# mandt-lab/PSLD

Hardware: NVIDIA B200
Metric: PSLD CIFAR-10 samples/sec (SSCS sampler) (higher is better)
Workload: dtype bf16x3

## Files before the change

### psld_b200/csrc/attn_tc.cu

```cuda

#include <cuda.h>

#include <new>

#include "common.cuh"
#include "tc_common.cuh"
#include "conv_tc_common.cuh"

namespace psld {

constexpr int AT_TILE = 128 * 64 * 2;
constexpr int AT_RING = 3;

template <bool kX3>
struct AtCfg {
  static constexpr int kMul = kX3 ? 2 : 1;
  static constexpr int kQP = 4 * AT_TILE * kMul;
  static constexpr int kSlot = AT_TILE * kMul;
  static constexpr int kParts = kX3 ? 2 : 1;
  static constexpr int kThreads = 64 + 128 * kParts;
  static constexpr int kXchg = kX3 ? 2048 : 0;
  static constexpr int kSmem = kQP + AT_RING * kSlot + 256 + kXchg;
  static constexpr int kMinBlocks = kX3 ? 1 : 2;
};

#ifdef PSLD_TC_TRACE
__device__ long long g_at_trace[1024 * 8];
#define AT_TRACE(slot) do { if ((threadIdx.x & 31) == 0) { const int b_ = blockIdx.y * gridDim.x + blockIdx.x; if (b_ < 1024) g_at_trace[b_ * 8 + (slot)] = clock64(); } } while (0)
#else
#define AT_TRACE(slot) do { } while (0)
#endif

struct AttnTcParams {
  __nv_bfloat16* out;
  int HW, C, N;
  int q_rows;
  int k_rows;
  int w_rows;
  float scale_log2;
  ConvTcParams ep;
};

struct AttnTcState {
  CUtensorMap tq, tkv, tw;
  bool proj, x3;
  AttnTcParams p;
  dim3 grid;
};

template <bool kProj, bool kX3>
__global__ void __launch_bounds__(AtCfg<kX3>::kThreads, AtCfg<kX3>::kMinBlocks)
attn_tc_kernel(const __grid_constant__ CUtensorMap tmQ, const __grid_constant__ CUtensorMap tmKV,
               const __grid_constant__ CUtensorMap tmW, const AttnTcParams p) {
  using Cfg = AtCfg<kX3>;
  constexpr uint32_t QP_LO = 4u * AT_TILE;
  constexpr uint32_t S_LO = AT_TILE;
  extern __shared__ uint8_t smem_raw[];
  pdl_trigger_early();
  if (threadIdx.x == 0) AT_TRACE(0);
  const uint32_t base = smem_u32(smem_raw);
  if (base & 1023u) __trap();
  const uint32_t qp = base;
  const uint32_t ring = base + Cfg::kQP;
  const uint32_t bar_base = ring + AT_RING * Cfg::kSlot;
  auto full_bar = [&](int s) { return bar_base + 8u * s; };
  auto empty_bar = [&](int s) { return bar_base + 8u * (AT_RING + s); };
  const uint32_t q_full = bar_base + 8u * (2 * AT_RING);
  const uint32_t s_full = q_full + 8u;
  const uint32_t p_ready = q_full + 16u;
  const uint32_t o_full = q_full + 24u;
  const uint32_t o_ready = q_full + 32u;
  const uint32_t y_full = q_full + 40u;
  const uint32_t tmem_slot = q_full + 48u;
  const uint32_t stg_base = ring;
  const uint32_t addv_base = ring + 8u * 4096u;
  constexpr int kParts = Cfg::kParts;
  float* xchg = reinterpret_cast<float*>(smem_raw + (bar_base + 256u - base));
  volatile uint32_t* tmem_slot_ptr =
      reinterpret_cast<volatile uint32_t*>(smem_raw + (tmem_slot - base));

  const int warp = threadIdx.x >> 5, lane = threadIdx.x & 31;
  const int n = blockIdx.y, q0 = blockIdx.x * 128;
  const int nck = p.C / 64;
  const int nkh = (p.HW + 127) / 128;
  const int nwt = (p.C + 127) / 128;
  const int lo_c = 3 * p.C;

  if (warp == 0 && lane == 0) {
    asm volatile("prefetch.tensormap [%0];" ::"l"(&tmQ) : "memory");
    asm volatile("prefetch.tensormap [%0];" ::"l"(&tmKV) : "memory");
    if (kProj) asm volatile("prefetch.tensormap [%0];" ::"l"(&tmW) : "memory");
    for (int s = 0; s < AT_RING; ++s) {
      mbar_init(full_bar(s), 1);
      mbar_init(empty_bar(s), 1);
    }
    mbar_init(q_full, 1);
    mbar_init(s_full, 1);
    mbar_init(p_ready, 128 * kParts);
    mbar_init(o_full, 1);
    mbar_init(o_ready, 128 * kParts);
    mbar_init(y_full, 1);
    asm volatile("fence.mbarrier_init.release.cluster;" ::: "memory");
  }
  if (warp == 1) {
    asm volatile("tcgen05.alloc.cta_group::1.sync.aligned.shared::cta.b32 [%0], %1;"
                 ::"r"(tmem_slot), "n"(256) : "memory");
    asm volatile("tcgen05.relinquish_alloc_permit.cta_group::1.sync.aligned;" ::: "memory");
  }
  tc_fence_before();
  __syncthreads();
  tc_fence_after();
  pdl_wait();
  const uint32_t tmem_acc = *tmem_slot_ptr;

  if (warp == 0) {
    if (lane == 0) {
      const uint32_t mul = kX3 ? 2u : 1u;
      mbar_arrive_expect_tx(q_full, (uint32_t)(nck * p.q_rows) * 128u * mul);
      for (int c = 0; c < nck; ++c) {
        tma_load_3d(qp + (uint32_t)c * AT_TILE, &tmQ, q_full, c * 64, q0, n);
        if (kX3) tma_load_3d(qp + QP_LO + (uint32_t)c * AT_TILE, &tmQ, q_full, lo_c + c * 64, q0, n);
      }
      int slot = 0;
      uint32_t phase = 0;
      auto next = [&]() { if (++slot == AT_RING) { slot = 0; phase ^= 1; } };
      for (int c = 0; c < nck; ++c)
        for (int h = 0; h < nkh; ++h) {
          mbar_wait(empty_bar(slot), phase ^ 1);
          mbar_arrive_expect_tx(full_bar(slot), (uint32_t)p.k_rows * 128u * mul);
          const uint32_t st = ring + (uint32_t)slot * Cfg::kSlot;
          tma_load_3d(st, &tmKV, full_bar(slot), p.C + c * 64, h * 128, n);
          if (kX3) tma_load_3d(st + S_LO, &tmKV, full_bar(slot), lo_c + p.C + c * 64, h * 128, n);
          next();
        }
      for (int g = 0; g < nck; ++g)
        for (int h = 0; h < nkh; ++h) {
          mbar_wait(empty_bar(slot), phase ^ 1);
          mbar_arrive_expect_tx(full_bar(slot), (uint32_t)p.k_rows * 128u * mul);
          const uint32_t st = ring + (uint32_t)slot * Cfg::kSlot;
          tma_load_3d(st, &tmKV, full_bar(slot), 2 * p.C + g * 64, h * 128, n);
          if (kX3) tma_load_3d(st + S_LO, &tmKV, full_bar(slot), lo_c + 2 * p.C + g * 64, h * 128, n);
          next();
        }
      if (kProj) {
        for (int c = 0; c < nck; ++c)
          for (int t = 0; t < nwt; ++t) {
            mbar_wait(empty_bar(slot), phase ^ 1);
            mbar_arrive_expect_tx(full_bar(slot), (uint32_t)p.w_rows * 128u * mul);
            const uint32_t st = ring + (uint32_t)slot * Cfg::kSlot;
            tma_load_2d(st, &tmW, full_bar(slot), c * 64, t * 128);
            if (kX3) tma_load_2d(st + S_LO, &tmW, full_bar(slot), c * 64, p.C + t * 128);
            next();
          }
      }
    }
  } else if (warp == 1) {
    if (lane == 0) {
      int slot = 0;
      uint32_t phase = 0;
      auto next = [&]() { if (++slot == AT_RING) { slot = 0; phase ^= 1; } };
      auto kgroup = [&](uint32_t d, uint32_t a_hi, uint32_t b_hi, uint32_t a_lo, uint32_t b_lo, uint32_t idesc,
                        bool first) {
        const uint64_t ad = make_sw128_desc(a_hi), bd = make_sw128_desc(b_hi);
#pragma unroll
        for (int k = 0; k < 4; ++k)
          tc_mma_bf16(d, ad + (uint64_t)(2 * k), bd + (uint64_t)(2 * k), idesc, (!first || k > 0) ? 1u : 0u);
        if (kX3) {
          const uint64_t al = make_sw128_desc(a_lo), bl = make_sw128_desc(b_lo);
#pragma unroll
          for (int k = 0; k < 4; ++k) tc_mma_bf16(d, ad + (uint64_t)(2 * k), bl + (uint64_t)(2 * k), idesc, 1u);
#pragma unroll
          for (int k = 0; k < 4; ++k) tc_mma_bf16(d, al + (uint64_t)(2 * k), bd + (uint64_t)(2 * k), idesc, 1u);
        }
      };
      const uint32_t idesc_s = (1u << 4) | (1u << 7) | (1u << 10) | ((uint32_t)(p.k_rows >> 3) << 17) |
                               ((uint32_t)(128 >> 4) << 24);
      mbar_wait(q_full, 0);
      tc_fence_after();
      AT_TRACE(1);
      for (int c = 0; c < nck; ++c)
        for (int h = 0; h < nkh; ++h) {
          mbar_wait(full_bar(slot), phase);
          tc_fence_after();
          const uint32_t st = ring + (uint32_t)slot * Cfg::kSlot;
          kgroup(tmem_acc + (uint32_t)h * 128u, qp + (uint32_t)c * AT_TILE, st,
                 qp + QP_LO + (uint32_t)c * AT_TILE, st + S_LO, idesc_s, c == 0);
          tc_commit(empty_bar(slot));
          next();
        }
      tc_commit(s_full);
      const uint32_t idesc_o = (1u << 4) | (1u << 7) | (1u << 10) | (1u << 16) |
                               ((uint32_t)(64 >> 3) << 17) | ((uint32_t)(128 >> 4) << 24);
      mbar_wait(p_ready, 0);
      tc_fence_after();
      for (int g = 0; g < nck; ++g)
        for (int h = 0; h < nkh; ++h) {
          mbar_wait(full_bar(slot), phase);
          tc_fence_after();
          const uint32_t st = ring + (uint32_t)slot * Cfg::kSlot;
          const uint32_t d = tmem_acc + (uint32_t)g * 64u;
          for (int ks = 0; ks < p.k_rows / 16; ++ks) {
            const int kg = h * 8 + ks;
            const uint32_t pa = qp + (uint32_t)(kg >> 2) * AT_TILE;
            const uint64_t adesc = make_sw128_desc(pa) + (uint64_t)(2 * (kg & 3));
            const uint64_t bdesc = make_sw128_desc(st + (uint32_t)ks * 2048u);
            tc_mma_bf16(d, adesc, bdesc, idesc_o, (h > 0 || ks > 0) ? 1u : 0u);
            if (kX3) {
              const uint64_t adesc_lo = make_sw128_desc(pa + QP_LO) + (uint64_t)(2 * (kg & 3));
              const uint64_t bdesc_lo = make_sw128_desc(st + S_LO + (uint32_t)ks * 2048u);
              tc_mma_bf16(d, adesc, bdesc_lo, idesc_o, 1u);
              tc_mma_bf16(d, adesc_lo, bdesc, idesc_o, 1u);
            }
          }
          tc_commit(empty_bar(slot));
          next();
        }
      tc_commit(o_full);
      if (kProj) {
        mbar_wait(o_ready, 0);
        tc_fence_after();
        for (int c = 0; c < nck; ++c)
          for (int t = 0; t < nwt; ++t) {
            mbar_wait(full_bar(slot), phase);
            tc_fence_after();
            const int rows = (p.C - t * 128) < 128 ? (p.C - t * 128) : 128;
            const uint32_t idesc_y = (1u << 4) | (1u << 7) | (1u << 10) | ((uint32_t)(rows >> 3) << 17) |
                                     ((uint32_t)(128 >> 4) << 24);
            const uint32_t st = ring + (uint32_t)slot * Cfg::kSlot;
            kgroup(tmem_acc + (uint32_t)t * 128u, qp + (uint32_t)c * AT_TILE, st,
                   qp + QP_LO + (uint32_t)c * AT_TILE, st + S_LO, idesc_y, c == 0);
            tc_commit(empty_bar(slot));
            next();
          }
        tc_commit(y_full);
      }
    }
  } else {
    const int quarter = warp & 3;
    const int row = quarter * 32 + lane;
    const uint32_t lane_addr = (uint32_t)(quarter * 32) << 16;
    const int part = kParts == 2 ? (warp >= 6 ? 1 : 0) : 0;
    const int k_lo = part * (p.HW / kParts), k_hi = k_lo + p.HW / kParts;
    const int c_lo = part * (p.C / kParts), c_hi = c_lo + p.C / kParts;
    auto pair_sync = [&]() {
      if (kParts == 2) asm volatile("bar.sync %0, 64;" ::"r"(2 + quarter) : "memory");
    };
    mbar_wait(s_full, 0);
    tc_fence_after();
    if (warp == 2) AT_TRACE(2);
    float mx = -INFINITY;
    for (int ch = k_lo; ch < k_hi; ch += 32) {
      uint32_t r[32];
      tmem_ld32(tmem_acc + lane_addr + (uint32_t)ch, r);
      tmem_ld_wait();
#pragma unroll
      for (int j = 0; j < 32; ++j) mx = fmaxf(mx, __uint_as_float(r[j]));
    }
    if (kParts == 2) {
      xchg[part * 128 + row] = mx;
      pair_sync();
      mx = fmaxf(mx, xchg[(part ^ 1) * 128 + row]);
    }
    const float mxs = mx * p.scale_log2;
    float sum = 0.f;
    for (int ch = k_lo; ch < k_hi; ch += 32) {
      uint32_t r[32];
      tmem_ld32(tmem_acc + lane_addr + (uint32_t)ch, r);
      tmem_ld_wait();
      const uint32_t tile = qp + (uint32_t)(ch >> 6) * AT_TILE + (uint32_t)row * 128u;
      const int cbase = (ch & 63) >> 3;
#pragma unroll
      for (int q = 0; q < 4; ++q) {
        uint32_t w[4], wl[4];
#pragma unroll
        for (int t = 0; t < 4; ++t) {
          const float e0 = exp2f(fmaf(__uint_as_float(r[q * 8 + 2 * t]), p.scale_log2, -mxs));
          const float e1 = exp2f(fmaf(__uint_as_float(r[q * 8 + 2 * t + 1]), p.scale_log2, -mxs));
          if (kX3) {
            split_bf2(e0, e1, w[t], wl[t]);
            sum += e0 + e1;
          } else {
            __nv_bfloat162 h = __floats2bfloat162_rn(e0, e1);
            const float2 f = __bfloat1622float2(h);
            sum += f.x + f.y;
            w[t] = *reinterpret_cast<uint32_t*>(&h);
          }
        }
        const uint32_t dst = tile + (uint32_t)(((cbase + q) ^ (row & 7)) << 4);
        sts128(dst, w[0], w[1], w[2], w[3]);
        if (kX3) sts128(dst + QP_LO, wl[0], wl[1], wl[2], wl[3]);
      }
    }
    asm volatile("fence.proxy.async.shared::cta;" ::: "memory");
    tc_fence_before();
    mbar_arrive(p_ready);
    if (warp == 2) AT_TRACE(3);
    if (kParts == 2) {
      xchg[256 + part * 128 + row] = sum;
      pair_sync();
      sum += xchg[256 + (part ^ 1) * 128 + row];
    }
    const float inv = 1.0f / sum;
    mbar_wait(o_full, 0);
    tc_fence_after();
    if (warp == 2) AT_TRACE(4);
    const int q = q0 + row;
    const bool valid = q < p.HW;
    if (kProj) {
      for (int ch = c_lo; ch < c_hi; ch += 32) {
        uint32_t r[32];
        tmem_ld32(tmem_acc + lane_addr + (uint32_t)ch, r);
        tmem_ld_wait();
        const uint32_t tile = qp + (uint32_t)(ch >> 6) * AT_TILE + (uint32_t)row * 128u;
        const int cbase = (ch & 63) >> 3;
#pragma unroll
        for (int j = 0; j < 4; ++j) {
          uint32_t w[4], wl[4];
#pragma unroll
          for (int t = 0; t < 4; ++t) {
            const float o0 = __uint_as_float(r[j * 8 + 2 * t]) * inv;
            const float o1 = __uint_as_float(r[j * 8 + 2 * t + 1]) * inv;
            if (kX3) split_bf2(o0, o1, w[t], wl[t]);
            else w[t] = f2_to_bf2(o0, o1);
          }
          const uint32_t dst = tile + (uint32_t)(((cbase + j) ^ (row & 7)) << 4);
          sts128(dst, w[0], w[1], w[2], w[3]);
          if (kX3) sts128(dst + QP_LO, wl[0], wl[1], wl[2], wl[3]);
        }
      }
      asm volatile("fence.proxy.async.shared::cta;" ::: "memory");
      tc_fence_before();
      mbar_arrive(o_ready);
      if (warp == 2) AT_TRACE(5);
      mbar_wait(y_full, 0);
      tc_fence_after();
      if (warp == 2) AT_TRACE(6);
      const int m_tile = n * (p.HW >> 7) + (int)blockIdx.x;
      const int ew = warp - 2;
#pragma unroll 1
      for (int half = (kParts == 2 ? part : 0); half < (kParts == 2 ? part + 1 : 2); ++half)
        tc_epilogue_tile<true, kX3 ? 32 : 64, !kX3, kX3>(p.ep, tmem_acc, 0, m_tile, 0, p.ep.block_n, quarter, half, lane,
                                                         stg_base + (uint32_t)ew * 4096u,
                                                         addv_base + (uint32_t)ew * 256u, []() {}, []() {});
    } else {
      __nv_bfloat16* orow = p.out + ((int64_t)n * p.HW + q) * (p.C * (kX3 ? 2 : 1));
      for (int ch = c_lo; ch < c_hi; ch += 32) {
        uint32_t r[32];
        tmem_ld32(tmem_acc + lane_addr + (uint32_t)ch, r);
        tmem_ld_wait();
        if (valid) {
#pragma unroll
          for (int j = 0; j < 32; j += 8) {
            uint32_t w[4], wl[4];
#pragma unroll
            for (int t = 0; t < 4; ++t) {
              const float o0 = __uint_as_float(r[j + 2 * t]) * inv;
              const float o1 = __uint_as_float(r[j + 2 * t + 1]) * inv;
              if (kX3) split_bf2(o0, o1, w[t], wl[t]);
              else w[t] = f2_to_bf2(o0, o1);
            }
            *reinterpret_cast<uint4*>(orow + ch + j) = make_uint4(w[0], w[1], w[2], w[3]);
            if (kX3) *reinterpret_cast<uint4*>(orow + p.C + ch + j) = make_uint4(wl[0], wl[1], wl[2], wl[3]);
          }
        }
        __syncwarp();
      }
    }
  }

  tc_fence_before();
  __syncthreads();
  if (threadIdx.x == 0) AT_TRACE(7);
  if (warp == 1) {
    tc_fence_after();
    asm volatile("tcgen05.dealloc.cta_group::1.sync.aligned.b32 %0, %1;"
                 ::"r"(tmem_acc), "n"(256) : "memory");
  }
}

#ifdef PSLD_TC_TRACE
extern "C" __attribute__((visibility("default"))) int psld_debug_attn_trace(long long* out) {
  return cudaMemcpyFromSymbol(out, g_at_trace, sizeof(g_at_trace)) == cudaSuccess ? 0 : 1;
}
#endif

static int encode_qkv_map(CUtensorMap* tm, const void* ptr, int N, int HW, int C3, int rows) {
  const cuuint64_t dims[3] = {(cuuint64_t)C3, (cuuint64_t)HW, (cuuint64_t)N};
  const cuuint64_t strides[2] = {(cuuint64_t)C3 * 2, (cuuint64_t)HW * C3 * 2};
  const cuuint32_t box[3] = {64, (cuuint32_t)rows, 1};
  const cuuint32_t estr[3] = {1, 1, 1};
  return encode_bf16_map(tm, ptr, 3, dims, strides, box, estr, "qkv");
}

int prepare_attn_tc(psld_op& op) {
  const int N = op.i[PSLD_ATTN_N], HW = op.i[PSLD_ATTN_HW], C = op.i[PSLD_ATTN_C];
  auto unsupported = [&](const char* why) {
    set_error("attn_tc: not eligible (%s): N=%d HW=%d C=%d", why, N, HW, C);
    return PSLD_EUNSUPPORTED;
  };
  const int adt = op.i[PSLD_ATTN_DTYPE];
  if (adt != PSLD_BF16 && adt != PSLD_BF16S) return unsupported("dtype must be bf16 or split bf16");
  const bool x3 = adt == PSLD_BF16S;
  const int cm = x3 ? 2 : 1;
  if (C % 64 || C < 64 || C > 256) return unsupported("C must be 64..256, multiple of 64");
  if (HW != 64 && HW != 128 && HW != 256) return unsupported("HW must be 64, 128 or 256");
  if (!op.in[0] || !op.out[0]) { set_error("attn_tc: null pointer"); return PSLD_EINVAL; }
  AttnTcState* st = new (std::nothrow) AttnTcState();
  if (!st) { set_error("attn_tc: out of host memory"); return PSLD_ECUDA; }
  const int q_rows = HW < 128 ? HW : 128;
  st->x3 = x3;
  int rc = encode_qkv_map(&st->tq, op.in[0], N, HW, cm * 3 * C, q_rows);
  if (rc == PSLD_OK) rc = encode_qkv_map(&st->tkv, op.in[0], N, HW, cm * 3 * C, q_rows);
  if (rc != PSLD_OK) { delete st; return rc; }
  st->p.out = (__nv_bfloat16*)op.out[0];
  st->p.HW = HW; st->p.C = C; st->p.N = N; st->p.q_rows = q_rows;
  st->p.k_rows = q_rows; st->p.w_rows = C < 128 ? C : 128;
  st->p.scale_log2 = op.f[0] * 1.4426950408889634f;
  st->grid = dim3((unsigned)((HW + 127) / 128), (unsigned)N);
  st->proj = op.i[PSLD_ATTN_PROJ] != 0;
  if (st->proj) {
    if (HW % 128 || !op.in[1] || !op.in[3]) { delete st; return unsupported("fused projection needs HW %% 128 == 0, weight and residual"); }
    rc = encode_w_map(&st->tw, op.in[1], cm * C, C, C < 128 ? C : 128);
    if (rc != PSLD_OK) { delete st; return rc; }
    ConvTcParams& e = st->p.ep;
    e = ConvTcParams{};
    e.bias = (const float*)op.in[2];
    e.temb = nullptr;
    e.res = (const __nv_bfloat16*)op.in[3];
    e.y = (__nv_bfloat16*)op.out[0];
    e.y_nchw = nullptr;
    e.mg_stats = (double*)op.out[1];
    e.cout_valid = C;
    e.scale = op.f[1];
    e.HW = HW; e.Cout = C; e.H = 0; e.W = 0;
    e.block_n = C; e.n_tiles_n = 1;
    e.M = (int64_t)N * HW;
  } else {
    st->tw = st->tq;
  }
  static bool attr_set = false;
  if (!attr_set) {
    cudaError_t e = cudaFuncSetAttribute(attn_tc_kernel<false, false>,
                                         cudaFuncAttributeMaxDynamicSharedMemorySize, AtCfg<false>::kSmem);
    if (e == cudaSuccess)
      e = cudaFuncSetAttribute(attn_tc_kernel<true, false>, cudaFuncAttributeMaxDynamicSharedMemorySize,
                               AtCfg<false>::kSmem);
    if (e == cudaSuccess)
      e = cudaFuncSetAttribute(attn_tc_kernel<false, true>, cudaFuncAttributeMaxDynamicSharedMemorySize,
                               AtCfg<true>::kSmem);
    if (e == cudaSuccess)
      e = cudaFuncSetAttribute(attn_tc_kernel<true, true>, cudaFuncAttributeMaxDynamicSharedMemorySize,
                               AtCfg<true>::kSmem);
    if (e == cudaSuccess)
      e = cudaFuncSetAttribute(attn_tc_kernel<false, false>, cudaFuncAttributePreferredSharedMemoryCarveout, 100);
    if (e == cudaSuccess)
      e = cudaFuncSetAttribute(attn_tc_kernel<true, false>, cudaFuncAttributePreferredSharedMemoryCarveout, 100);
    if (e != cudaSuccess) {
      set_error("attn_tc: cudaFuncSetAttribute failed: %s", cudaGetErrorString(e));
      delete st;
      return PSLD_ECUDA;
    }
    attr_set = true;
  }
  op.aux = st;
  return PSLD_OK;
}

int release_attn_tc(psld_op& op) {
  if (op.aux) {
    delete (AttnTcState*)op.aux;
    op.aux = nullptr;
  }
  return PSLD_OK;
}

int run_attn_tc(const psld_op& op, cudaStream_t s) {
  const AttnTcState* st = (const AttnTcState*)op.aux;
  PSLD_CHECK_ARG(st != nullptr, "attn_tc: op not prepared (call psld_op_prepare)");
#define ATTN_LAUNCH(PROJ, X3)                                                                  \
  PSLD_CHECK_CUDA(launch_pdl(attn_tc_kernel<PROJ, X3>, st->grid, dim3(AtCfg<X3>::kThreads),       \
                             AtCfg<X3>::kSmem, s, 1, st->tq, st->tkv,                              \
                             st->tw, st->p))
  if (st->proj) { if (st->x3) ATTN_LAUNCH(true, true); else ATTN_LAUNCH(true, false); }
  else { if (st->x3) ATTN_LAUNCH(false, true); else ATTN_LAUNCH(false, false); }
#undef ATTN_LAUNCH
  PSLD_CHECK_LAUNCH();
  return PSLD_OK;
}

}
```

Baseline: 5.508.

## Make bf16x3 attention kernel persistent with double-buffered TMEM and dedicated epilogue warps

Turns the split-bf16 attention kernel into a persistent kernel that loops over (batch, query-tile) units, with the grid capped at the SM count. TMEM accumulators are double-buffered so the next unit's QK^T and PV MMAs can run while four dedicated epilogue warps finish the fused projection, residual add and statistics of the previous unit. Q reuse is guarded by a new barrier. This replaces the earlier two-part softmax warp split, aiming to hide epilogue and launch latency, but it adds barrier complexity and can unbalance load when there are few units.

```diff
diff --git a/psld_b200/csrc/attn_tc.cu b/psld_b200/csrc/attn_tc.cu
--- a/psld_b200/csrc/attn_tc.cu
+++ b/psld_b200/csrc/attn_tc.cu
@@ -1,6 +1,7 @@
 
 #include <cuda.h>
 
+#include <algorithm>
 #include <new>
 
 #include "common.cuh"
@@ -10,25 +11,28 @@
 namespace psld {
 
 constexpr int AT_TILE = 128 * 64 * 2;
-constexpr int AT_RING = 3;
 
 template <bool kX3>
 struct AtCfg {
+  static constexpr bool kPersist = kX3;
   static constexpr int kMul = kX3 ? 2 : 1;
   static constexpr int kQP = 4 * AT_TILE * kMul;
   static constexpr int kSlot = AT_TILE * kMul;
-  static constexpr int kParts = kX3 ? 2 : 1;
-  static constexpr int kThreads = 64 + 128 * kParts;
-  static constexpr int kXchg = kX3 ? 2048 : 0;
-  static constexpr int kSmem = kQP + AT_RING * kSlot + 256 + kXchg;
-  static constexpr int kMinBlocks = kX3 ? 1 : 2;
+  static constexpr int kRing = 3;
+  static constexpr int kWin = kPersist ? 2 : 1;
+  static constexpr int kEpiWarps = kPersist ? 4 : 0;
+  static constexpr int kThreads = 64 + 128 + 32 * kEpiWarps;
+  static constexpr int kSmem = kQP + kRing * kSlot + 256;
+  static constexpr int kMinBlocks = kPersist ? 1 : 2;
 };
+static_assert(AtCfg<true>::kSmem <= 227 * 1024, "bf16x3 attention shared-memory plan exceeds 227 KB");
+static_assert(2 * AtCfg<false>::kSmem <= 227 * 1024, "bf16 attention must fit two CTAs per SM");
 
 #ifdef PSLD_TC_TRACE
 __device__ long long g_at_trace[1024 * 8];
-#define AT_TRACE(slot) do { if ((threadIdx.x & 31) == 0) { const int b_ = blockIdx.y * gridDim.x + blockIdx.x; if (b_ < 1024) g_at_trace[b_ * 8 + (slot)] = clock64(); } } while (0)
+#define AT_TRACE(unit, slot) do { if ((threadIdx.x & 31) == 0 && (unit) < 1024) g_at_trace[(unit) * 8 + (slot)] = clock64(); } while (0)
 #else
-#define AT_TRACE(slot) do { } while (0)
+#define AT_TRACE(unit, slot) do { } while (0)
 #endif
 
 struct AttnTcParams {
@@ -37,6 +41,7 @@
   int q_rows;
   int k_rows;
   int w_rows;
+  int units;
   float scale_log2;
   ConvTcParams ep;
 };
@@ -48,117 +53,206 @@
   dim3 grid;
 };
 
+template <class Release>
+__device__ __forceinline__ void attn_row_epilogue(const ConvTcParams& p, uint32_t tmem_acc, int m_tile,
+                                                  int quarter, int lane, Release release) {
+  const int64_t m_base = (int64_t)m_tile * 128 + quarter * 32;
+  const int64_t ldo = 2 * (int64_t)p.Cout;
+  const __nv_bfloat16* rrow = p.res + (m_base + lane) * ldo;
+  __nv_bfloat16* yrow = p.y + (m_base + lane) * ldo;
+  const float scale = p.scale;
+  const uint32_t taddr = tmem_acc + ((uint32_t)(quarter * 32) << 16);
+  uint4 rh[4], rl[4];
+  auto load_res = [&](int co0) {
+#pragma unroll
+    for (int t = 0; t < 4; ++t) {
+      rh[t] = *reinterpret_cast<const uint4*>(rrow + co0 + 8 * t);
+      rl[t] = *reinterpret_cast<const uint4*>(rrow + p.Cout + co0 + 8 * t);
+    }
+  };
+  load_res(0);
+#pragma unroll 1
+  for (int co0 = 0; co0 < p.Cout; co0 += 32) {
+    uint32_t r[32];
+    tmem_ld32(taddr + (uint32_t)co0, r);
+    float v[32];
+#pragma unroll
+    for (int q = 0; q < 4; ++q) {
+      const uint32_t hw[4] = {rh[q].x, rh[q].y, rh[q].z, rh[q].w};
+      const uint32_t lw[4] = {rl[q].x, rl[q].y, rl[q].z, rl[q].w};
+#pragma unroll
+      for (int t = 0; t < 4; ++t) {
+        const float2 f = __bfloat1622float2(*reinterpret_cast<const __nv_bfloat162*>(&hw[t]));
+        const float2 g = __bfloat1622float2(*reinterpret_cast<const __nv_bfloat162*>(&lw[t]));
+        v[q * 8 + 2 * t] = f.x + g.x;
+        v[q * 8 + 2 * t + 1] = f.y + g.y;
+      }
+    }
+    if (co0 + 32 < p.Cout) load_res(co0 + 32);
+    tmem_ld_wait();
+    if (co0 + 32 >= p.Cout) release();
+#pragma unroll
+    for (int j = 0; j < 32; j += 4) {
+      const float4 b = p.bias ? __ldg(reinterpret_cast<const float4*>(p.bias + co0 + j)) : make_float4(0.f, 0.f, 0.f, 0.f);
+      const float bb[4] = {b.x, b.y, b.z, b.w};
+#pragma unroll
+      for (int k = 0; k < 4; ++k)
+        v[j + k] = fmaf(v[j + k], scale, fmaf(__uint_as_float(r[j + k]), scale, bb[k] * scale));
+    }
+#pragma unroll
+    for (int q = 0; q < 4; ++q) {
+      uint32_t o[4], ol[4];
+#pragma unroll
+      for (int t = 0; t < 4; ++t) split_bf2(v[q * 8 + 2 * t], v[q * 8 + 2 * t + 1], o[t], ol[t]);
+      *reinterpret_cast<uint4*>(yrow + co0 + 8 * q) = make_uint4(o[0], o[1], o[2], o[3]);
+      *reinterpret_cast<uint4*>(yrow + p.Cout + co0 + 8 * q) = make_uint4(ol[0], ol[1], ol[2], ol[3]);
+    }
+    if (p.mg_stats) {
+      float a[16];
+#pragma unroll
+      for (int g = 0; g < 8; ++g) {
+        const float x0 = v[4 * g], x1 = v[4 * g + 1], x2 = v[4 * g + 2], x3 = v[4 * g + 3];
+        a[2 * g] = (x0 + x1) + (x2 + x3);
+        a[2 * g + 1] = fmaf(x0, x0, fmaf(x1, x1, fmaf(x2, x2, x3 * x3)));
+      }
+#pragma unroll
+      for (int w = 8; w >= 1; w >>= 1) {
+        const bool hi = (lane & (2 * w)) != 0;
+#pragma unroll
+        for (int j = 0; j < w; ++j) {
+          const float send = hi ? a[j] : a[j + w];
+          const float keep = hi ? a[j + w] : a[j];
+          a[j] = keep + __shfl_xor_sync(0xffffffffu, send, 2 * w);
+        }
+      }
+      a[0] += __shfl_xor_sync(0xffffffffu, a[0], 1);
+      if ((lane & 1) == 0)
+        atomicAdd(p.mg_stats + ((m_base / p.HW) * (p.Cout >> 2) + (co0 >> 2)) * 2 + (lane >> 1), (double)a[0]);
+    }
+  }
+}
+
 template <bool kProj, bool kX3>
 __global__ void __launch_bounds__(AtCfg<kX3>::kThreads, AtCfg<kX3>::kMinBlocks)
 attn_tc_kernel(const __grid_constant__ CUtensorMap tmQ, const __grid_constant__ CUtensorMap tmKV,
                const __grid_constant__ CUtensorMap tmW, const AttnTcParams p) {
   using Cfg = AtCfg<kX3>;
+  constexpr int kRing = Cfg::kRing, kWin = Cfg::kWin;
   constexpr uint32_t QP_LO = 4u * AT_TILE;
   constexpr uint32_t S_LO = AT_TILE;
   extern __shared__ uint8_t smem_raw[];
   pdl_trigger_early();
-  if (threadIdx.x == 0) AT_TRACE(0);
   const uint32_t base = smem_u32(smem_raw);
   if (base & 1023u) __trap();
   const uint32_t qp = base;
   const uint32_t ring = base + Cfg::kQP;
-  const uint32_t bar_base = ring + AT_RING * Cfg::kSlot;
+  const uint32_t stg_base = ring;
+  const uint32_t addv_base = ring + 8u * 4096u;
+  const uint32_t bar_base = ring + kRing * Cfg::kSlot;
   auto full_bar = [&](int s) { return bar_base + 8u * s; };
-  auto empty_bar = [&](int s) { return bar_base + 8u * (AT_RING + s); };
-  const uint32_t q_full = bar_base + 8u * (2 * AT_RING);
+  auto empty_bar = [&](int s) { return bar_base + 8u * (kRing + s); };
+  const uint32_t q_full = bar_base + 8u * (2 * kRing);
   const uint32_t s_full = q_full + 8u;
   const uint32_t p_ready = q_full + 16u;
   const uint32_t o_full = q_full + 24u;
   const uint32_t o_ready = q_full + 32u;
-  const uint32_t y_full = q_full + 40u;
-  const uint32_t tmem_slot = q_full + 48u;
-  const uint32_t stg_base = ring;
-  const uint32_t addv_base = ring + 8u * 4096u;
-  constexpr int kParts = Cfg::kParts;
-  float* xchg = reinterpret_cast<float*>(smem_raw + (bar_base + 256u - base));
+  const uint32_t qp_free = q_full + 40u;
+  auto y_full = [&](int w) { return q_full + 48u + 8u * w; };
+  auto win_free = [&](int w) { return q_full + 64u + 8u * w; };
+  const uint32_t tmem_slot = q_full + 80u;
   volatile uint32_t* tmem_slot_ptr =
       reinterpret_cast<volatile uint32_t*>(smem_raw + (tmem_slot - base));
 
   const int warp = threadIdx.x >> 5, lane = threadIdx.x & 31;
-  const int n = blockIdx.y, q0 = blockIdx.x * 128;
+  constexpr int epi_warp0 = 6;
   const int nck = p.C / 64;
   const int nkh = (p.HW + 127) / 128;
   const int nwt = (p.C + 127) / 128;
   const int lo_c = 3 * p.C;
+  if (threadIdx.x == 0) AT_TRACE((int)blockIdx.x, 0);
 
   if (warp == 0 && lane == 0) {
     asm volatile("prefetch.tensormap [%0];" ::"l"(&tmQ) : "memory");
     asm volatile("prefetch.tensormap [%0];" ::"l"(&tmKV) : "memory");
     if (kProj) asm volatile("prefetch.tensormap [%0];" ::"l"(&tmW) : "memory");
-    for (int s = 0; s < AT_RING; ++s) {
+    for (int s = 0; s < kRing; ++s) {
       mbar_init(full_bar(s), 1);
       mbar_init(empty_bar(s), 1);
     }
     mbar_init(q_full, 1);
     mbar_init(s_full, 1);
-    mbar_init(p_ready, 128 * kParts);
+    mbar_init(p_ready, 128);
     mbar_init(o_full, 1);
-    mbar_init(o_ready, 128 * kParts);
-    mbar_init(y_full, 1);
+    mbar_init(o_ready, 128);
+    mbar_init(qp_free, 1);
+    for (int w = 0; w < 2; ++w) {
+      mbar_init(y_full(w), 1);
+      mbar_init(win_free(w), 128);
+    }
     asm volatile("fence.mbarrier_init.release.cluster;" ::: "memory");
   }
   if (warp == 1) {
     asm volatile("tcgen05.alloc.cta_group::1.sync.aligned.shared::cta.b32 [%0], %1;"
-                 ::"r"(tmem_slot), "n"(256) : "memory");
+                 ::"r"(tmem_slot), "n"(256 * kWin) : "memory");
     asm volatile("tcgen05.relinquish_alloc_permit.cta_group::1.sync.aligned;" ::: "memory");
   }
   tc_fence_before();
   __syncthreads();
   tc_fence_after();
   pdl_wait();
-  const uint32_t tmem_acc = *tmem_slot_ptr;
+  const uint32_t tmem_base = *tmem_slot_ptr;
 
   if (warp == 0) {
     if (lane == 0) {
       const uint32_t mul = kX3 ? 2u : 1u;
-      mbar_arrive_expect_tx(q_full, (uint32_t)(nck * p.q_rows) * 128u * mul);
-      for (int c = 0; c < nck; ++c) {
-        tma_load_3d(qp + (uint32_t)c * AT_TILE, &tmQ, q_full, c * 64, q0, n);
-        if (kX3) tma_load_3d(qp + QP_LO + (uint32_t)c * AT_TILE, &tmQ, q_full, lo_c + c * 64, q0, n);
-      }
       int slot = 0;
       uint32_t phase = 0;
-      auto next = [&]() { if (++slot == AT_RING) { slot = 0; phase ^= 1; } };
-      for (int c = 0; c < nck; ++c)
-        for (int h = 0; h < nkh; ++h) {
-          mbar_wait(empty_bar(slot), phase ^ 1);
-          mbar_arrive_expect_tx(full_bar(slot), (uint32_t)p.k_rows * 128u * mul);
-          const uint32_t st = ring + (uint32_t)slot * Cfg::kSlot;
-          tma_load_3d(st, &tmKV, full_bar(slot), p.C + c * 64, h * 128, n);
-          if (kX3) tma_load_3d(st + S_LO, &tmKV, full_bar(slot), lo_c + p.C + c * 64, h * 128, n);
-          next();
-        }
-      for (int g = 0; g < nck; ++g)
-        for (int h = 0; h < nkh; ++h) {
-          mbar_wait(empty_bar(slot), phase ^ 1);
-          mbar_arrive_expect_tx(full_bar(slot), (uint32_t)p.k_rows * 128u * mul);
-          const uint32_t st = ring + (uint32_t)slot * Cfg::kSlot;
-          tma_load_3d(st, &tmKV, full_bar(slot), 2 * p.C + g * 64, h * 128, n);
-          if (kX3) tma_load_3d(st + S_LO, &tmKV, full_bar(slot), lo_c + 2 * p.C + g * 64, h * 128, n);
-          next();
-        }
-      if (kProj) {
+      auto next = [&]() { if (++slot == kRing) { slot = 0; phase ^= 1; } };
+      int i = 0;
+      for (int u = blockIdx.x; u < p.units; u += gridDim.x, ++i) {
+        const int n = u / nkh, q0 = (u - n * nkh) * 128;
+        if (i > 0) mbar_wait(qp_free, (i - 1) & 1);
+        mbar_arrive_expect_tx(q_full, (uint32_t)(nck * p.q_rows) * 128u * mul);
+        for (int c = 0; c < nck; ++c) {
+          tma_load_3d(qp + (uint32_t)c * AT_TILE, &tmQ, q_full, c * 64, q0, n);
+          if (kX3) tma_load_3d(qp + QP_LO + (uint32_t)c * AT_TILE, &tmQ, q_full, lo_c + c * 64, q0, n);
+        }
         for (int c = 0; c < nck; ++c)
-          for (int t = 0; t < nwt; ++t) {
+          for (int h = 0; h < nkh; ++h) {
             mbar_wait(empty_bar(slot), phase ^ 1);
-            mbar_arrive_expect_tx(full_bar(slot), (uint32_t)p.w_rows * 128u * mul);
+            mbar_arrive_expect_tx(full_bar(slot), (uint32_t)p.k_rows * 128u * mul);
             const uint32_t st = ring + (uint32_t)slot * Cfg::kSlot;
-            tma_load_2d(st, &tmW, full_bar(slot), c * 64, t * 128);
-            if (kX3) tma_load_2d(st + S_LO, &tmW, full_bar(slot), c * 64, p.C + t * 128);
+            tma_load_3d(st, &tmKV, full_bar(slot), p.C + c * 64, h * 128, n);
+            if (kX3) tma_load_3d(st + S_LO, &tmKV, full_bar(slot), lo_c + p.C + c * 64, h * 128, n);
             next();
           }
+        for (int g = 0; g < nck; ++g)
+          for (int h = 0; h < nkh; ++h) {
+            mbar_wait(empty_bar(slot), phase ^ 1);
+            mbar_arrive_expect_tx(full_bar(slot), (uint32_t)p.k_rows * 128u * mul);
+            const uint32_t st = ring + (uint32_t)slot * Cfg::kSlot;
+            tma_load_3d(st, &tmKV, full_bar(slot), 2 * p.C + g * 64, h * 128, n);
+            if (kX3) tma_load_3d(st + S_LO, &tmKV, full_bar(slot), lo_c + 2 * p.C + g * 64, h * 128, n);
+            next();
+          }
+        if (kProj) {
+          for (int c = 0; c < nck; ++c)
+            for (int t = 0; t < nwt; ++t) {
+              mbar_wait(empty_bar(slot), phase ^ 1);
+              mbar_arrive_expect_tx(full_bar(slot), (uint32_t)p.w_rows * 128u * mul);
+              const uint32_t st = ring + (uint32_t)slot * Cfg::kSlot;
+              tma_load_2d(st, &tmW, full_bar(slot), c * 64, t * 128);
+              if (kX3) tma_load_2d(st + S_LO, &tmW, full_bar(slot), c * 64, p.C + t * 128);
+              next();
+            }
+        }
       }
     }
   } else if (warp == 1) {
     if (lane == 0) {
       int slot = 0;
       uint32_t phase = 0;
-      auto next = [&]() { if (++slot == AT_RING) { slot = 0; phase ^= 1; } };
+      auto next = [&]() { if (++slot == kRing) { slot = 0; phase ^= 1; } };
       auto kgroup = [&](uint32_t d, uint32_t a_hi, uint32_t b_hi, uint32_t a_lo, uint32_t b_lo, uint32_t idesc,
                         bool first) {
         const uint64_t ad = make_sw128_desc(a_hi), bd = make_sw128_desc(b_hi);
@@ -175,206 +269,222 @@
       };
       const uint32_t idesc_s = (1u << 4) | (1u << 7) | (1u << 10) | ((uint32_t)(p.k_rows >> 3) << 17) |
                                ((uint32_t)(128 >> 4) << 24);
-      mbar_wait(q_full, 0);
-      tc_fence_after();
-      AT_TRACE(1);
-      for (int c = 0; c < nck; ++c)
-        for (int h = 0; h < nkh; ++h) {
-          mbar_wait(full_bar(slot), phase);
-          tc_fence_after();
-          const uint32_t st = ring + (uint32_t)slot * Cfg::kSlot;
-          kgroup(tmem_acc + (uint32_t)h * 128u, qp + (uint32_t)c * AT_TILE, st,
-                 qp + QP_LO + (uint32_t)c * AT_TILE, st + S_LO, idesc_s, c == 0);
-          tc_commit(empty_bar(slot));
-          next();
-        }
-      tc_commit(s_full);
       const uint32_t idesc_o = (1u << 4) | (1u << 7) | (1u << 10) | (1u << 16) |
                                ((uint32_t)(64 >> 3) << 17) | ((uint32_t)(128 >> 4) << 24);
-      mbar_wait(p_ready, 0);
-      tc_fence_after();
-      for (int g = 0; g < nck; ++g)
-        for (int h = 0; h < nkh; ++h) {
-          mbar_wait(full_bar(slot), phase);
-          tc_fence_after();
-          const uint32_t st = ring + (uint32_t)slot * Cfg::kSlot;
-          const uint32_t d = tmem_acc + (uint32_t)g * 64u;
-          for (int ks = 0; ks < p.k_rows / 16; ++ks) {
-            const int kg = h * 8 + ks;
-            const uint32_t pa = qp + (uint32_t)(kg >> 2) * AT_TILE;
-            const uint64_t adesc = make_sw128_desc(pa) + (uint64_t)(2 * (kg & 3));
-            const uint64_t bdesc = make_sw128_desc(st + (uint32_t)ks * 2048u);
-            tc_mma_bf16(d, adesc, bdesc, idesc_o, (h > 0 || ks > 0) ? 1u : 0u);
-            if (kX3) {
-              const uint64_t adesc_lo = make_sw128_desc(pa + QP_LO) + (uint64_t)(2 * (kg & 3));
-              const uint64_t bdesc_lo = make_sw128_desc(st + S_LO + (uint32_t)ks * 2048u);
-              tc_mma_bf16(d, adesc, bdesc_lo, idesc_o, 1u);
-              tc_mma_bf16(d, adesc_lo, bdesc, idesc_o, 1u);
-            }
-          }
-          tc_commit(empty_bar(slot));
-          next();
-        }
-      tc_commit(o_full);
-      if (kProj) {
-        mbar_wait(o_ready, 0);
+      int i = 0;
+      for (int u = blockIdx.x; u < p.units; u += gridDim.x, ++i) {
+        const int w = i % kWin;
+        const uint32_t tmem_acc = tmem_base + (uint32_t)w * 256u;
+        if (i >= kWin) mbar_wait(win_free(w), ((i / kWin) - 1) & 1);
+        mbar_wait(q_full, i & 1);
         tc_fence_after();
+        AT_TRACE(u, 1);
         for (int c = 0; c < nck; ++c)
-          for (int t = 0; t < nwt; ++t) {
+          for (int h = 0; h < nkh; ++h) {
             mbar_wait(full_bar(slot), phase);
             tc_fence_after();
-            const int rows = (p.C - t * 128) < 128 ? (p.C - t * 128) : 128;
-            const uint32_t idesc_y = (1u << 4) | (1u << 7) | (1u << 10) | ((uint32_t)(rows >> 3) << 17) |
-                                     ((uint32_t)(128 >> 4) << 24);
             const uint32_t st = ring + (uint32_t)slot * Cfg::kSlot;
-            kgroup(tmem_acc + (uint32_t)t * 128u, qp + (uint32_t)c * AT_TILE, st,
-                   qp + QP_LO + (uint32_t)c * AT_TILE, st + S_LO, idesc_y, c == 0);
+            kgroup(tmem_acc + (uint32_t)h * 128u, qp + (uint32_t)c * AT_TILE, st,
+                   qp + QP_LO + (uint32_t)c * AT_TILE, st + S_LO, idesc_s, c == 0);
             tc_commit(empty_bar(slot));
             next();
           }
-        tc_commit(y_full);
-      }
-    }
-  } else {
+        tc_commit(s_full);
+        mbar_wait(p_ready, i & 1);
+        tc_fence_after();
+        for (int g = 0; g < nck; ++g)
+          for (int h = 0; h < nkh; ++h) {
+            mbar_wait(full_bar(slot), phase);
+            tc_fence_after();
+            const uint32_t st = ring + (uint32_t)slot * Cfg::kSlot;
+            const uint32_t d = tmem_acc + (uint32_t)g * 64u;
+            for (int ks = 0; ks < p.k_rows / 16; ++ks) {
+              const int kg = h * 8 + ks;
+              const uint32_t pa = qp + (uint32_t)(kg >> 2) * AT_TILE;
+              const uint64_t adesc = make_sw128_desc(pa) + (uint64_t)(2 * (kg & 3));
+              const uint64_t bdesc = make_sw128_desc(st + (uint32_t)ks * 2048u);
+              tc_mma_bf16(d, adesc, bdesc, idesc_o, (h > 0 || ks > 0) ? 1u : 0u);
+              if (kX3) {
+                const uint64_t adesc_lo = make_sw128_desc(pa + QP_LO) + (uint64_t)(2 * (kg & 3));
+                const uint64_t bdesc_lo = make_sw128_desc(st + S_LO + (uint32_t)ks * 2048u);
+                tc_mma_bf16(d, adesc, bdesc_lo, idesc_o, 1u);
+                tc_mma_bf16(d, adesc_lo, bdesc, idesc_o, 1u);
+              }
+            }
+            tc_commit(empty_bar(slot));
+            next();
+          }
+        tc_commit(o_full);
+        if (kProj) {
+          mbar_wait(o_ready, i & 1);
+          tc_fence_after();
+          for (int c = 0; c < nck; ++c)
+            for (int t = 0; t < nwt; ++t) {
+              mbar_wait(full_bar(slot), phase);
+              tc_fence_after();
+              const int rows = (p.C - t * 128) < 128 ? (p.C - t * 128) : 128;
+              const uint32_t idesc_y = (1u << 4) | (1u << 7) | (1u << 10) | ((uint32_t)(rows >> 3) << 17) |
+                                       ((uint32_t)(128 >> 4) << 24);
+              const uint32_t st = ring + (uint32_t)slot * Cfg::kSlot;
+              kgroup(tmem_acc + (uint32_t)t * 128u, qp + (uint32_t)c * AT_TILE, st,
+                     qp + QP_LO + (uint32_t)c * AT_TILE, st + S_LO, idesc_y, c == 0);
+              tc_commit(empty_bar(slot));
+              next();
+            }
+          tc_commit(qp_free);
+          tc_commit(y_full(w));
+        } else {
+          tc_commit(qp_free);
+        }
+      }
+    }
+  } else if (warp < epi_warp0) {
     const int quarter = warp & 3;
     const int row = quarter * 32 + lane;
     const uint32_t lane_addr = (uint32_t)(quarter * 32) << 16;
-    const int part = kParts == 2 ? (warp >= 6 ? 1 : 0) : 0;
-    const int k_lo = part * (p.HW / kParts), k_hi = k_lo + p.HW / kParts;
-    const int c_lo = part * (p.C / kParts), c_hi = c_lo + p.C / kParts;
-    auto pair_sync = [&]() {
-      if (kParts == 2) asm volatile("bar.sync %0, 64;" ::"r"(2 + quarter) : "memory");
-    };
-    mbar_wait(s_full, 0);
-    tc_fence_after();
-    if (warp == 2) AT_TRACE(2);
-    float mx = -INFINITY;
-    for (int ch = k_lo; ch < k_hi; ch += 32) {
-      uint32_t r[32];
-      tmem_ld32(tmem_acc + lane_addr + (uint32_t)ch, r);
-      tmem_ld_wait();
-#pragma unroll
-      for (int j = 0; j < 32; ++j) mx = fmaxf(mx, __uint_as_float(r[j]));
-    }
-    if (kParts == 2) {
-      xchg[part * 128 + row] = mx;
-      pair_sync();
-      mx = fmaxf(mx, xchg[(part ^ 1) * 128 + row]);
-    }
-    const float mxs = mx * p.scale_log2;
-    float sum = 0.f;
-    for (int ch = k_lo; ch < k_hi; ch += 32) {
-      uint32_t r[32];
-      tmem_ld32(tmem_acc + lane_addr + (uint32_t)ch, r);
-      tmem_ld_wait();
-      const uint32_t tile = qp + (uint32_t)(ch >> 6) * AT_TILE + (uint32_t)row * 128u;
-      const int cbase = (ch & 63) >> 3;
-#pragma unroll
-      for (int q = 0; q < 4; ++q) {
-        uint32_t w[4], wl[4];
-#pragma unroll
-        for (int t = 0; t < 4; ++t) {
-          const float e0 = exp2f(fmaf(__uint_as_float(r[q * 8 + 2 * t]), p.scale_log2, -mxs));
-          const float e1 = exp2f(fmaf(__uint_as_float(r[q * 8 + 2 * t + 1]), p.scale_log2, -mxs));
-          if (kX3) {
-            split_bf2(e0, e1, w[t], wl[t]);
-            sum += e0 + e1;
-          } else {
-            __nv_bfloat162 h = __floats2bfloat162_rn(e0, e1);
-            const float2 f = __bfloat1622float2(h);
-            sum += f.x + f.y;
-            w[t] = *reinterpret_cast<uint32_t*>(&h);
-          }
-        }
-        const uint32_t dst = tile + (uint32_t)(((cbase + q) ^ (row & 7)) << 4);
-        sts128(dst, w[0], w[1], w[2], w[3]);
-        if (kX3) sts128(dst + QP_LO, wl[0], wl[1], wl[2], wl[3]);
-      }
-    }
-    asm volatile("fence.proxy.async.shared::cta;" ::: "memory");
-    tc_fence_before();
-    mbar_arrive(p_ready);
-    if (warp == 2) AT_TRACE(3);
-    if (kParts == 2) {
-      xchg[256 + part * 128 + row] = sum;
-      pair_sync();
-      sum += xchg[256 + (part ^ 1) * 128 + row];
-    }
-    const float inv = 1.0f / sum;
-    mbar_wait(o_full, 0);
-    tc_fence_after();
-    if (warp == 2) AT_TRACE(4);
-    const int q = q0 + row;
-    const bool valid = q < p.HW;
-    if (kProj) {
-      for (int ch = c_lo; ch < c_hi; ch += 32) {
+    int i = 0;
+    for (int u = blockIdx.x; u < p.units; u += gridDim.x, ++i) {
+      const int w = i % kWin;
+      const uint32_t tmem_acc = tmem_base + (uint32_t)w * 256u;
+      const int n = u / nkh, q0 = (u - n * nkh) * 128;
+      mbar_wait(s_full, i & 1);
+      tc_fence_after();
+      if (warp == 2) AT_TRACE(u, 2);
+      float mx = -INFINITY;
+      for (int ch = 0; ch < p.HW; ch += 32) {
+        uint32_t r[32];
+        tmem_ld32(tmem_acc + lane_addr + (uint32_t)ch, r);
+        tmem_ld_wait();
+#pragma unroll
+        for (int j = 0; j < 32; ++j) mx = fmaxf(mx, __uint_as_float(r[j]));
+      }
+      const float mxs = mx * p.scale_log2;
+      float sum = 0.f;
+      for (int ch = 0; ch < p.HW; ch += 32) {
         uint32_t r[32];
         tmem_ld32(tmem_acc + lane_addr + (uint32_t)ch, r);
         tmem_ld_wait();
         const uint32_t tile = qp + (uint32_t)(ch >> 6) * AT_TILE + (uint32_t)row * 128u;
         const int cbase = (ch & 63) >> 3;
 #pragma unroll
-        for (int j = 0; j < 4; ++j) {
-          uint32_t w[4], wl[4];
+        for (int q = 0; q < 4; ++q) {
+          uint32_t wv[4], wl[4];
 #pragma unroll
           for (int t = 0; t < 4; ++t) {
-            const float o0 = __uint_as_float(r[j * 8 + 2 * t]) * inv;
-            const float o1 = __uint_as_float(r[j * 8 + 2 * t + 1]) * inv;
-            if (kX3) split_bf2(o0, o1, w[t], wl[t]);
-            else w[t] = f2_to_bf2(o0, o1);
+            const float e0 = exp2f(fmaf(__uint_as_float(r[q * 8 + 2 * t]), p.scale_log2, -mxs));
+            const float e1 = exp2f(fmaf(__uint_as_float(r[q * 8 + 2 * t + 1]), p.scale_log2, -mxs));
+            if (kX3) {
+              split_bf2(e0, e1, wv[t], wl[t]);
+              sum += e0 + e1;
+            } else {
+              __nv_bfloat162 h = __floats2bfloat162_rn(e0, e1);
+              const float2 f = __bfloat1622float2(h);
+              sum += f.x + f.y;
+              wv[t] = *reinterpret_cast<uint32_t*>(&h);
+            }
           }
-          const uint32_t dst = tile + (uint32_t)(((cbase + j) ^ (row & 7)) << 4);
-          sts128(dst, w[0], w[1], w[2], w[3]);
+          const uint32_t dst = tile + (uint32_t)(((cbase + q) ^ (row & 7)) << 4);
+          sts128(dst, wv[0], wv[1], wv[2], wv[3]);
           if (kX3) sts128(dst + QP_LO, wl[0], wl[1], wl[2], wl[3]);
         }
       }
       asm volatile("fence.proxy.async.shared::cta;" ::: "memory");
       tc_fence_before();
-      mbar_arrive(o_ready);
-      if (warp == 2) AT_TRACE(5);
-      mbar_wait(y_full, 0);
+      mbar_arrive(p_ready);
+      if (warp == 2) AT_TRACE(u, 3);
+      const float inv = 1.0f / sum;
+      mbar_wait(o_full, i & 1);
       tc_fence_after();
-      if (warp == 2) AT_TRACE(6);
-      const int m_tile = n * (p.HW >> 7) + (int)blockIdx.x;
-      const int ew = warp - 2;
+      if (warp == 2) AT_TRACE(u, 4);
+      const int q = q0 + row;
+      const bool valid = q < p.HW;
+      if (kProj) {
+        for (int ch = 0; ch < p.C; ch += 32) {
+          uint32_t r[32];
+          tmem_ld32(tmem_acc + lane_addr + (uint32_t)ch, r);
+          tmem_ld_wait();
+          const uint32_t tile = qp + (uint32_t)(ch >> 6) * AT_TILE + (uint32_t)row * 128u;
+          const int cbase = (ch & 63) >> 3;
+#pragma unroll
+          for (int j = 0; j < 4; ++j) {
+            uint32_t wv[4], wl[4];
+#pragma unroll
+            for (int t = 0; t < 4; ++t) {
+              const float o0 = __uint_as_float(r[j * 8 + 2 * t]) * inv;
+              const float o1 = __uint_as_float(r[j * 8 + 2 * t + 1]) * inv;
+              if (kX3) split_bf2(o0, o1, wv[t], wl[t]);
+              else wv[t] = f2_to_bf2(o0, o1);
+            }
+            const uint32_t dst = tile + (uint32_t)(((cbase + j) ^ (row & 7)) << 4);
+            sts128(dst, wv[0], wv[1], wv[2], wv[3]);
+            if (kX3) sts128(dst + QP_LO, wl[0], wl[1], wl[2], wl[3]);
+          }
+        }
+        asm volatile("fence.proxy.async.shared::cta;" ::: "memory");
+        tc_fence_before();
+        mbar_arrive(o_ready);
+        if (warp == 2) AT_TRACE(u, 5);
+        if (!Cfg::kPersist) {
+          mbar_wait(y_full(0), 0);
+          tc_fence_after();
+          if (warp == 2) AT_TRACE(u, 6);
 #pragma unroll 1
-      for (int half = (kParts == 2 ? part : 0); half < (kParts == 2 ? part + 1 : 2); ++half)
-        tc_epilogue_tile<true, kX3 ? 32 : 64, !kX3, kX3>(p.ep, tmem_acc, 0, m_tile, 0, p.ep.block_n, quarter, half, lane,
-                                                         stg_base + (uint32_t)ew * 4096u,
-                                                         addv_base + (uint32_t)ew * 256u, []() {}, []() {});
-    } else {
-      __nv_bfloat16* orow = p.out + ((int64_t)n * p.HW + q) * (p.C * (kX3 ? 2 : 1));
-      for (int ch = c_lo; ch < c_hi; ch += 32) {
-        uint32_t r[32];
-        tmem_ld32(tmem_acc + lane_addr + (uint32_t)ch, r);
-        tmem_ld_wait();
-        if (valid) {
-#pragma unroll
-          for (int j = 0; j < 32; j += 8) {
-            uint32_t w[4], wl[4];
-#pragma unroll
-            for (int t = 0; t < 4; ++t) {
-              const float o0 = __uint_as_float(r[j + 2 * t]) * inv;
-              const float o1 = __uint_as_float(r[j + 2 * t + 1]) * inv;
-              if (kX3) split_bf2(o0, o1, w[t], wl[t]);
-              else w[t] = f2_to_bf2(o0, o1);
+          for (int half = 0; half < 2; ++half)
+            tc_epilogue_tile<true, 64, true, false>(p.ep, tmem_acc, 0, u, 0, p.ep.block_n, quarter, half, lane,
+                                                    stg_base + (uint32_t)(warp - 2) * 4096u,
+                                                    addv_base + (uint32_t)(warp - 2) * 256u, []() {}, []() {});
+          if (warp == 2) AT_TRACE(u, 7);
+        }
+      } else {
+        __nv_bfloat16* orow = p.out + ((int64_t)n * p.HW + q) * (p.C * (kX3 ? 2 : 1));
+        for (int ch = 0; ch < p.C; ch += 32) {
+          uint32_t r[32];
+          tmem_ld32(tmem_acc + lane_addr + (uint32_t)ch, r);
+          tmem_ld_wait();
+          if (valid) {
+#pragma unroll
+            for (int j = 0; j < 32; j += 8) {
+              uint32_t wv[4], wl[4];
+#pragma unroll
+              for (int t = 0; t < 4; ++t) {
+                const float o0 = __uint_as_float(r[j + 2 * t]) * inv;
+                const float o1 = __uint_as_float(r[j + 2 * t + 1]) * inv;
+                if (kX3) split_bf2(o0, o1, wv[t], wl[t]);
+                else wv[t] = f2_to_bf2(o0, o1);
+              }
+              *reinterpret_cast<uint4*>(orow + ch + j) = make_uint4(wv[0], wv[1], wv[2], wv[3]);
+              if (kX3) *reinterpret_cast<uint4*>(orow + p.C + ch + j) = make_uint4(wl[0], wl[1], wl[2], wl[3]);
             }
-            *reinterpret_cast<uint4*>(orow + ch + j) = make_uint4(w[0], w[1], w[2], w[3]);
-            if (kX3) *reinterpret_cast<uint4*>(orow + p.C + ch + j) = make_uint4(wl[0], wl[1], wl[2], wl[3]);
           }
-        }
-        __syncwarp();
-      }
+          __syncwarp();
+        }
+        tc_fence_before();
+        mbar_arrive(win_free(w));
+        if (warp == 2) AT_TRACE(u, 7);
+      }
+    }
+  } else if (kProj) {
+    const int quarter = warp & 3;
+    const int ew = warp - epi_warp0;
+    int i = 0;
+    for (int u = blockIdx.x; u < p.units; u += gridDim.x, ++i) {
+      const int w = i % kWin;
+      mbar_wait(y_full(w), (i / kWin) & 1);
+      tc_fence_after();
+      if (ew == 0) AT_TRACE(u, 6);
+      const uint32_t tmem_acc = tmem_base + (uint32_t)w * 256u;
+      const uint32_t wf = win_free(w);
+      attn_row_epilogue(p.ep, tmem_acc, u, quarter, lane, [&]() { tc_fence_before(); mbar_arrive(wf); });
+      if (ew == 0) AT_TRACE(u, 7);
     }
   }
 
   tc_fence_before();
   __syncthreads();
-  if (threadIdx.x == 0) AT_TRACE(7);
   if (warp == 1) {
     tc_fence_after();
     asm volatile("tcgen05.dealloc.cta_group::1.sync.aligned.b32 %0, %1;"
-                 ::"r"(tmem_acc), "n"(256) : "memory");
+                 ::"r"(tmem_base), "n"(256 * kWin) : "memory");
   }
 }
 
@@ -416,7 +526,9 @@
   st->p.HW = HW; st->p.C = C; st->p.N = N; st->p.q_rows = q_rows;
   st->p.k_rows = q_rows; st->p.w_rows = C < 128 ? C : 128;
   st->p.scale_log2 = op.f[0] * 1.4426950408889634f;
-  st->grid = dim3((unsigned)((HW + 127) / 128), (unsigned)N);
+  st->p.units = N * ((HW + 127) / 128);
+  const bool persist = x3 ? AtCfg<true>::kPersist : AtCfg<false>::kPersist;
+  st->grid = dim3((unsigned)(persist ? std::min(st->p.units, sm_count()) : st->p.units));
   st->proj = op.i[PSLD_ATTN_PROJ] != 0;
   if (st->proj) {
     if (HW % 128 || !op.in[1] || !op.in[3]) { delete st; return unsupported("fused projection needs HW %% 128 == 0, weight and residual"); }
```

New measurement: 5.507, median of 6. No clear change (-0.0%).
